# Jiraiya812/Fast-CU-Decision-HEVC

Measured on AMD Instinct MI355X. Metric: CTUs/sec (RDO decision only) at 4K all-intra, higher is better.
Workload: dtype int32+f64

## Files before the change

### fast-cu-decision-hevc_amd/csrc/fcu_engine.h

```cpp
#pragma once
#include <stdint.h>
#include <string.h>
#include <type_traits>
#include "../../include/fcu.h"

#ifdef FCU_EMU
#include <math.h>
#include <stdio.h>
#include <stdlib.h>
#define FCU_DEV static inline
#define FCU_MEMBER inline
#define FCU_NOINLINE
#define FCU_INLINE
#define FCU_TABLE static const
static int g_emu_phase = 0, g_emu_in_phase = 0, g_emu_lane = 0, g_emu_relax = 0;
#define FCU_EMU_RELAX(on) (g_emu_relax = (on))
static inline int fcu_emu_phase_begin() { g_emu_phase++; g_emu_in_phase = 1; g_emu_lane = 0; return 0; }
static inline int fcu_emu_phase_next(int lane) { if (lane + 1 >= 64) g_emu_in_phase = 0; g_emu_lane = lane + 1; return lane + 1; }
template <class T> static inline T fcu_emu_uni(T v, int site, int line)
{
  enum { SITES = 2048, K = 32, B = 16 };
  struct Seen { int phase, first, cur, idx, n; unsigned char vals[K][B]; };
  static Seen seen[SITES];
  if (g_emu_in_phase && !g_emu_relax && sizeof(T) <= B && site < SITES) {
// ... 37 lines not shown
  v += (uint32_t)__builtin_amdgcn_update_dpp(0, (int)v, 0x143, 0xc, 0xf, false);
  return (uint32_t)__builtin_amdgcn_readlane((int)v, 63);
}
__device__ inline unsigned long long fcu_wave_min64(unsigned long long v)
{
  for (int o = 32; o > 0; o >>= 1) {
    const unsigned lo = (unsigned)__shfl_xor((int)(unsigned)v, o), hi = (unsigned)__shfl_xor((int)(unsigned)(v >> 32), o);
    const unsigned long long w = ((unsigned long long)hi << 32) | lo;
    v = w < v ? w : v;
  }
  return v;
}
#define FCU_WAVE_ADD(p, v) do { const uint32_t s_ = fcu_wave_sum(v); if (threadIdx.x == 0) *(p) += s_; } while (0)
#define FCU_WAVE_MIN64(p, v) do { const unsigned long long s_ = fcu_wave_min64(v); if (threadIdx.x == 0 && s_ < *(p)) *(p) = s_; } while (0)
template <class T> __device__ inline T fcu_uni(T v)
{
  static_assert(sizeof(T) % 4 == 0, "dword-sized objects only");
  int w[sizeof(T) / 4];
  __builtin_memcpy(w, &v, sizeof(T));
  for (unsigned i = 0; i < sizeof(T) / 4; i++) w[i] = __builtin_amdgcn_readfirstlane(w[i]);
  __builtin_memcpy(&v, w, sizeof(T));
  return v;
}
#define FCU_UNI(x) fcu_uni(x)
#define FCU_EMU_RELAX(on) do { } while (0)
#if defined(__HIP_DEVICE_COMPILE__)
#define FCU_HBM __attribute__((address_space(1)))
#else
#define FCU_HBM
#endif
#define FCU_GENERIC_(p) ((const __attribute__((address_space(0))) void *)(p))
#define FCU_IN_LDS(p) __builtin_assume(__builtin_amdgcn_is_shared(FCU_GENERIC_(p)))
#define FCU_FLOOR(x) floor(x)
#define FCU_CHECK(c) do { } while (0)
#endif
#define FCU_DIST_ADD(acc, v, e, i, n2) do { \
    if ((n2) >= 64) { (acc) += (uint32_t)((e) * (e)); if (((((i) - lane) + 64) & ((n2) - 1)) == 0) { FCU_WAVE_ADD(&g_S.vc_dist[v], acc); (acc) = 0; } } \
    else FCU_ATOMIC_ADD(&g_S.vc_dist[v], (uint32_t)((e) * (e))); } while (0)
#define FCU_SERIAL FCU_FOR_LANES if (lane == 0)
#if defined(FCU_PROFILE) && !defined(FCU_EMU)
#define FCU_TIC(v) const long long v = clock64()
#ifdef FCU_PROFILE_RQT
#define FCU_QTIC(v) long long v = clock64()
#define FCU_QTOC(E_, v, idx) do { if (threadIdx.x == 0) (E_).C->prof[idx] += (unsigned long long)(clock64() - v); v = clock64(); } while (0)
#define FCU_TOC(E_, v, idx) do { if ((idx) == 10 && threadIdx.x == 0) (E_).C->prof[idx] += (unsigned long long)(clock64() - v); } while (0)
#define FCU_COUNT(E_, idx, n) do { } while (0)
#elif defined(FCU_PROFILE_INTER)
#define FCU_ITOC(E_, v, idx) do { if (threadIdx.x == 0) (E_).C->prof[idx] += (unsigned long long)(clock64() - v); } while (0)
#define FCU_TOC(E_, v, idx) do { if ((idx) == 10 && threadIdx.x == 0) (E_).C->prof[idx] += (unsigned long long)(clock64() - v); } while (0)
#define FCU_COUNT(E_, idx, n) do { } while (0)
#elif defined(FCU_PROFILE_RDOQ) || defined(FCU_PROFILE_DEPTH)
#define FCU_TOC(E_, v, idx) do { if ((idx) < 11 && threadIdx.x == 0) (E_).C->prof[idx] += (unsigned long long)(clock64() - v); } while (0)
#define FCU_COUNT(E_, idx, n) do { } while (0)
#else
#define FCU_TOC(E_, v, idx) do { if (threadIdx.x == 0) (E_).C->prof[idx] += (unsigned long long)(clock64() - v); } while (0)
#define FCU_COUNT(E_, idx, n) do { (E_).C->prof[idx] += (unsigned long long)(n); } while (0)
#endif
#else
#define FCU_TIC(v) do { } while (0)
#define FCU_TOC(E_, v, idx) do { } while (0)
#define FCU_COUNT(E_, idx, n) do { } while (0)
#endif
#ifndef FCU_QTOC
#define FCU_QTIC(v) do { } while (0)
#define FCU_QTOC(E_, v, idx) do { } while (0)
#endif
#ifndef FCU_ITOC
#define FCU_ITOC(E_, v, idx) do { } while (0)
#endif

#include "fcu_tables.h"

struct HotTables { uint32_t bin[256]; uint16_t scan[3][16]; uint8_t scan_cg8[3][4]; uint8_t ctx_ind_map4x4[16]; uint8_t group_idx[32];
                   uint64_t scan4_nib[3], map4_nib; uint32_t cnt_bits[4]; };
#ifdef FCU_EMU
static HotTables g_hot;
#else
__shared__ HotTables g_hot;
#endif

#if defined(FCU_PROFILE_RQT) && !defined(FCU_EMU)
#define FCU_RTIC(v) long long v = clock64()
#define FCU_RTOC(P_, v, idx) do { if (!SER && threadIdx.x == 0) { ((Chain *)((char *)&(P_) - __builtin_offsetof(Chain, p)))->prof[idx] += (unsigned long long)(clock64() - v); v = clock64(); } } while (0)
#elif defined(FCU_PROFILE_RDOQ) && !defined(FCU_EMU)
#define FCU_RTIC(v) long long v = clock64()
#define FCU_RTOC(P_, v, idx) do { if (SER) { ((Chain *)((char *)&(P_) - __builtin_offsetof(Chain, p)))->prof[idx] += (unsigned long long)(clock64() - v); v = clock64(); } } while (0)
#else
#define FCU_RTIC(v) do { } while (0)
#define FCU_RTOC(P_, v, idx) do { } while (0)
#endif
namespace fcu {

enum { CTU = 64, MAXDEPTH = 3, NPART = 256, LOG2_MAXTU = 5, LOG2_MINTU = 2, TU_MAXDEPTH_INTRA = 3 };
enum { SIZE_2Nx2N = 0, SIZE_2NxN = 1, SIZE_Nx2N = 2, SIZE_NxN = 3, SIZE_2NxnU = 4, SIZE_2NxnD = 5, SIZE_nLx2N = 6, SIZE_nRx2N = 7, SIZE_NONE = 8, MODE_INTER = 0, MODE_INTRA = 1, MODE_NONE = 2 };
enum { SLICE_I = 0, SLICE_P = 1 };
enum { PLANAR = 0, DC = 1, HOR = 10, VER = 26, DM_CHROMA = 36 };
enum { CTX_SPLIT = 0, CTX_PARTSIZE = 3, CTX_INTRA_LUMA = 4, CTX_CHROMA_PRED = 5, CTX_CBF_LUMA = 6, CTX_CBF_CHROMA = 11,
       CTX_SUBDIV = 16, CTX_SIGCG = 19, CTX_SIG = 23, CTX_LASTX = 67, CTX_LASTY = 97, CTX_ONE = 127, CTX_ABS = 151,
       CTX_TSKIP = 157, NCTX_INTRA = 160,
       CTX_SKIP = 160, CTX_MERGE_FLAG = 163, CTX_MERGE_IDX = 164, CTX_PRED_MODE = 165, CTX_PARTSIZE1 = 166, CTX_MVD = 169,
       CTX_REF = 171, CTX_MVP_IDX = 173, CTX_ROOT_CBF = 174, NCTX = 176 };
enum { CI_CURR_BEST = 0, CI_NEXT_BEST, CI_TEMP_BEST, CI_CHROMA_INTRA, CI_QT_TRAFO_TEST, CI_QT_TRAFO_ROOT, CI_NUM };
enum { MEMO_K = 6, MEMO_POOL = 6144 + 1536 + 384 + 96 };
enum { MAXVC = 20, MAXLC = 16, POOL = 5120 };
#define FCU_MAX_DOUBLE 1.7e+308

struct Cabac { uint8_t ctx[NCTX]; uint64_t frac; uint32_t bins; uint32_t pad_; };

struct Params {
  int width, height, qp, qp_c, slice_ctus, slice_type;
  int transform_skip, ts_fast, sign_hiding, strong_smoothing;
  double lambda, sqrt_lambda, chroma_weight, rdoq_lambda[3];
  double err_scale[2][4];
  long long rd_factor[2];
  int search_range, fast_enc, had_me, fdm, max_merge_cand, fast_search;
  int tmvp;
  int amp;
  int rdoq, rdoq_ts;
  uint32_t lambda_motion_sad;
  int cabac_b_table;
};
// ... 43 lines not shown
struct Yuv { uint8_t y[64 * 64], u[32 * 32], v[32 * 32]; };
enum { FCU_REF_MARGIN = 80 };
struct ChromaModeBuf { uint8_t u[32 * 32], v[32 * 32]; alignas(16) int16_t coef[2][1024]; uint8_t cbf[2][NPART], tskip[2][NPART]; };

struct RdoqRec { double cc, cs, c0; int32_t up, dn, sd, du; };

struct alignas(16) Scratch {
  CuObj cu[4][2];
  Yuv org[4], predt[4], reco[4][2];
  Yuv qt_rec[4];
  alignas(16) int16_t qt_coef[3][4][CTU * CTU];
  int16_t ts_coef[3][1024]; Yuv ts_rec; uint8_t shared_pred[3][1024];
  uint8_t tmp_tr_idx[NPART], tmp_cbf[NPART], tmp_tskip[NPART];
  ChromaModeBuf cm[5];
  Cabac slots[MAXDEPTH + 2][CI_NUM];
  uint8_t p_pred[POOL]; int16_t p_resi[POOL]; int32_t p_tmp[POOL]; int32_t p_tcoef[POOL]; uint8_t p_rec[POOL];
  int32_t p_lscan[POOL]; int16_t p_qscan[POOL];
  RdoqRec r_rec[POOL]; double r_cg[MAXVC * 64];
  uint8_t c64_rec[5][CTU * CTU]; alignas(16) int16_t c64_coef[5][CTU * CTU];
  Cabac c64_state[5][4]; uint32_t c64_distk[5][4];
  Yuv16 resi_cu, resi_best, qt_resi[4];
  Yuv tmp_pred;
  uint8_t me_pred[9][CTU * CTU];
  int16_t me_h[3][72 * 64];
  int par_ps[4];
  int memo_valid[4][MEMO_K], memo_next[4], memo_zero[4][MEMO_K];
  int16_t memo_mv[4][MEMO_K][NPART][2]; int8_t memo_ref[4][MEMO_K][NPART];
  uint8_t memo_tr_idx[4][MEMO_K][NPART], memo_cbf[4][MEMO_K][3][NPART], memo_tskip[4][MEMO_K][3][NPART];
  alignas(16) int16_t memo_coef[MEMO_K * MEMO_POOL], memo_resi[MEMO_K * MEMO_POOL];
};

struct Env { Chain *C; Scratch *G; int cur_ctu, slice_start; };
struct TU { int log2, tr_depth, part, nparts, x, y, off_y, cw, cwo, cx, cy, c_tr_depth, c_code_all, off_c, cu_depth, plast; };

struct Shared {
  Cabac cab[1 + (MAXDEPTH + 1) + MAXLC];
  uint8_t ref5[5][68]; int dc5[5]; uint32_t cm_dist[5];
  union {
    int16_t lane_abs[MAXLC][32];
    RdoqRec rq_rec[16];
    struct {
      int32_t colsum[128];
      union {
        struct { uint8_t ref[264], reff[264]; };
        uint8_t ref5b[5][68];
      };
    };
  };
  union {
    int16_t rq_lv[16];
    uint32_t sad[36];
  };
  int dc;
  int best_idx[4], reco_best_idx[4];
  union {
    struct { int rd_mode[12]; int n_rd; int preds[3]; int n_mpm; };
    int uni[8];
  };
  union {
    struct {
      uint8_t vc_slot[MAXVC];
      int vc_abs[MAXVC], vc_lsp[MAXVC], vc_last[MAXVC]; uint32_t vc_dist[MAXVC]; uint32_t vc_bits[MAXVC]; double vc_cost[MAXVC];
    };
    struct {
      uint32_t acc[16];
      unsigned long long me_best;
      int mrg_mv[5][2], mrg_ref[5], amvp[2][2];
      int iv_abs[6], iv_lsp[6], iv_top[6]; uint32_t iv_dist[6], iv_bits[6];
      int it_abs[3], it_ts[3]; uint32_t it_dist[3];
      double iq_cost[5]; uint32_t iq_bits[5], iq_dist[5], iq_zero;
      int16_t tz_x[16], tz_y[16]; uint8_t tz_pt[16], tz_d[16]; int tz_n;
      uint32_t tz_best; int tz_bx, tz_by, tz_dist, tz_round, tz_point;
      int mrg_buf[5], best_is_skip, me_out[4];
    };
  };
  int pu_best_vc, pu_best_mode, pu_nvc; uint32_t pu_best_dist; double pu_best_cost;
  int t_abs, t_lsp, t_last; uint32_t t_dist;
  int rw_abs, rw_lsp;
  double q_cost[4]; uint32_t q_dist[4];
  int c_best_mode; uint32_t c_best_dist; double c_best_cost; int c_modes[5];
  uint32_t c_dist;
  Env env;
  TU wk_st[4]; int wk_ci[4]; int wk_part[4], wk_child[4];
  double cand_cost[12];
  uint32_t c64_dist[5]; uint8_t c64_cbf[5][4]; int c64_valid;
  uint64_t q_frac[5], t_frac;
  double dec_j0, dec_j1; int dec_cnt, dec_flip;
};

enum { CAB_GOON = 0, CAB_CUR0 = 1, CAB_LANE0 = 1 + (MAXDEPTH + 1) };
enum { EST_CODERS = 7 };
static_assert(EST_CODERS * sizeof(Cabac) >= NCTX_INTRA * 2 * sizeof(uint32_t) && EST_CODERS <= MAXLC, "est table does not fit its lane coders");
#define FCU_EST ((uint32_t *)&g_S.cab[CAB_LANE0 + MAXLC - EST_CODERS])
#ifdef FCU_EMU
static Shared g_S;
#else
__shared__ Shared g_S;
#endif
FCU_DEV Env env_get() { return FCU_UNI(g_S.env); }
FCU_DEV Cabac *slot_ptr(const Env E, int d, int ci) { return ci == CI_CURR_BEST ? &g_S.cab[CAB_CUR0 + d] : &E.G->slots[d][ci]; }


FCU_DEV int part_x(int z) { return (k_z2r[z] & 15) << 2; }
FCU_DEV int part_y(int z) { return (k_z2r[z] >> 4) << 2; }
FCU_DEV int zidx_of(int lx, int ly) { return k_r2z[((ly & 63) >> 2) * 16 + ((lx & 63) >> 2)]; }
FCU_DEV int ilog2(int n) { int l = 0; while ((1 << l) < n) l++; return l; }
FCU_DEV int iabs(int v) { return v < 0 ? -v : v; }
FCU_DEV int clip8(int v) { return v < 0 ? 0 : (v > 255 ? 255 : v); }
FCU_DEV int clip3i(int lo, int hi, int v) { return v < lo ? lo : (v > hi ? hi : v); }
FCU_DEV uint8_t *yuv_plane(Yuv *b, int comp) { return comp == 0 ? b->y : (comp == 1 ? b->u : b->v); }
FCU_DEV double rd_cost(const Params &p, uint32_t bits, uint32_t dist)
{ return FCU_FLOOR((double)dist + ((double)bits * p.lambda) + 0.5); }

FCU_DEV void tu_root(TU &t, int depth)
{
  t.log2 = 6 - depth; t.tr_depth = 0; t.part = 0; t.nparts = NPART >> (2 * depth); t.x = t.y = 0; t.off_y = 0;
  t.cw = t.cwo = (CTU >> depth) >> 1; t.cx = t.cy = 0; t.c_tr_depth = 0; t.c_code_all = 1; t.off_c = 0;
  t.cu_depth = depth; t.plast = 0;
}
FCU_DEV void tu_child(TU &c, const TU &p, int i, int processLast)
{
  const int s = 1 << (p.log2 - 1);
  c.log2 = p.log2 - 1; c.tr_depth = p.tr_depth + 1; c.cu_depth = p.cu_depth; c.plast = processLast;
  c.nparts = p.nparts >> 2; if (c.nparts < 1) c.nparts = 1;
  c.part = p.part + i * c.nparts;
  c.x = p.x + (i & 1) * s; c.y = p.y + (i >> 1) * s; c.off_y = p.off_y + i * s * s;
  const int pw = p.cwo;
  if ((pw >> 1) >= 4) {
    const int cs = pw >> 1;
    c.cw = c.cwo = cs; c.c_code_all = 1; c.c_tr_depth = p.c_tr_depth + 1;
    c.cx = p.cx + (i & 1) * cs; c.cy = p.cy + (i >> 1) * cs; c.off_c = p.off_c + i * cs * cs;
  } else {
    c.cwo = pw; c.c_code_all = 0; c.c_tr_depth = p.c_tr_depth; c.cx = p.cx; c.cy = p.cy; c.off_c = p.off_c;
    c.cw = (processLast ? (i == 3) : (i == 0)) ? pw : 0;
  }
}
FCU_DEV uint32_t tu_key(const TU &t) { return (uint32_t)(t.cu_depth | (t.tr_depth << 2) | (t.part << 4) | (t.plast << 12)); }
FCU_DEV TU tu_of_key(uint32_t k)
{
  TU t; tu_root(t, (int)(k & 3));
  const int trd = (int)((k >> 2) & 3), part = (int)((k >> 4) & 255), pl = (int)((k >> 12) & 1);
  for (int l = 0; l < trd; l++) {
    TU c; int np = t.nparts >> 2; if (np < 1) np = 1;
    tu_child(c, t, ((part - t.part) / np) & 3, pl);
    t = c;
  }
// ... 916 lines not shown
  const int N = 1 << log2;
  const uint8_t *corner = ref + 2 * N;
  if (mode == PLANAR)
    return ((N - 1 - x) * corner[-1 - y] + (x + 1) * corner[1 + N] + (N - 1 - y) * corner[1 + x] + (y + 1) * corner[-1 - N] + N) >> (log2 + 1);
  if (mode == DC) {
    int v = dc;
    if (isLuma && N <= 16) {
      if (x == 0 && y == 0) v = (corner[1] + corner[-1] + 2 * dc + 2) >> 2;
      else if (y == 0) v = (corner[1 + x] + 3 * dc + 2) >> 2;
      else if (x == 0) v = (corner[-1 - y] + 3 * dc + 2) >> 2;
    }
    return v;
  }
  const int isVer = mode >= 18;
  const int angMode = isVer ? mode - VER : -(mode - HOR);
  const int absAng = iabs(angMode);
  const int angAbs = (int)((0x2069544d245080ull >> (6 * absAng)) & 63);
  const int invAngle = absAng == 0 ? 0 : (int)(((absAng <= 4 ? 0x13b0e38ccd000ull : 0x8004ec30c1e2ull) >> (13 * ((absAng - 1) & 3))) & 8191);
  const int angle = angMode < 0 ? -angAbs : angAbs;
  const int px = isVer ? x : y, py = isVer ? y : x, ms = isVer ? 1 : -1;
  if (angle == 0) {
    int v = corner[ms * (px + 1)];
    if (isLuma && N <= 16 && px == 0) v = clip8(v + ((corner[-ms * (py + 1)] - corner[0]) >> 1));
    return v;
  }
  const int deltaPos = (py + 1) * angle, di = deltaPos >> 5, df = deltaPos & 31;
  const int i0 = px + di + 1;
  int r0, r1;
  { int i = i0; r0 = (i >= 0) ? corner[ms * i] : corner[-ms * ((128 + (-i) * invAngle) >> 8)]; }
  if (!df) return r0;
  { int i = i0 + 1; r1 = (i >= 0) ? corner[ms * i] : corner[-ms * ((128 + (-i) * invAngle) >> 8)]; }
  return ((32 - df) * r0 + df * r1 + 16) >> 5;
}

FCU_DEV int unit_available(const Env E, int lx, int ly, int cx, int cy)
{
  const Params &P = E.C->p;
  if (lx < 0 || ly < 0 || lx >= P.width || ly >= P.height) return 0;
  const int ctuN = (ly >> 6) * E.C->w_ctu + (lx >> 6), ctuC = (cy >> 6) * E.C->w_ctu + (cx >> 6);
  if (ctuN < E.slice_start) return 0;
  if (ctuN < ctuC) return 1;
  if (ctuN > ctuC) return 0;
  return zidx_of(lx, ly) < zidx_of(cx, cy);
}

FCU_DEV FCU_NOINLINE void build_ref(int comp, int px, int py, int log2, int wantFilt)
{
  const Env E = env_get(); comp = FCU_UNI(comp); px = FCU_UNI(px); py = FCU_UNI(py); log2 = FCU_UNI(log2); wantFilt = FCU_UNI(wantFilt);
  const int N = 1 << log2, sh = comp ? 1 : 0, unit = 4 >> sh, total = 4 * N + 1;
  const int lx0 = px << sh, ly0 = py << sh;
  const uint8_t *rec = E.C->rec[comp]; const int stride = E.C->stride[comp];
  uint8_t *ref = g_S.ref, *avail = (uint8_t *)g_S.colsum;
  FCU_FOR_LANES {
    for (int i = lane; i < total; i += 64) {
      int a, v = 0;
      if (i < 2 * N) { const int y = 2 * N - 1 - i; a = unit_available(E, lx0 - 4, ((py + y) / unit * unit) << sh, lx0, ly0); if (a) v = rec[(py + y) * stride + px - 1]; }
      else if (i == 2 * N) { a = unit_available(E, lx0 - 4, ly0 - 4, lx0, ly0); if (a) v = rec[(py - 1) * stride + px - 1]; }
      else { const int x = i - 2 * N - 1; a = unit_available(E, ((px + x) / unit * unit) << sh, ly0 - 4, lx0, ly0); if (a) v = rec[(py - 1) * stride + px + x]; }
      avail[i] = (uint8_t)a; ref[i] = (uint8_t)v;
    }
  }
  FCU_FOR_LANES {
    for (int i = lane; i < total; i += 64) {
      if (!avail[i]) {
        int j = i - 1;
        while (j >= 0 && !avail[j]) j--;
        if (j < 0) { j = i + 1; while (j < total && !avail[j]) j++; }
        g_S.reff[i] = (j < total) ? ref[j] : 128;
      }
    }
  }
  FCU_FOR_LANES { for (int i = lane; i < total; i += 64) if (!avail[i]) ref[i] = g_S.reff[i]; }
  FCU_FOR_LANES {
    if (lane == 0) { int sum = 0; for (int i = 0; i < N; i++) sum += ref[2 * N + 1 + i] + ref[2 * N - 1 - i]; g_S.dc = (sum + N) >> (log2 + 1); }
    if (wantFilt) {
      int strong = 0;
      if (comp == 0 && E.C->p.strong_smoothing && N >= 32) {
        const int bl = ref[0], tl = ref[2 * N], tr = ref[4 * N];
        strong = (iabs(bl + tl - 2 * ref[N]) < 8) && (iabs(tl + tr - 2 * ref[3 * N]) < 8);
      }
      for (int i = lane; i < total; i += 64) {
        int v;
        if (i == 0 || i == 4 * N) v = ref[i];
        else if (strong) {
          const int bl = ref[0], tl = ref[2 * N], tr = ref[4 * N];
          if (i < 2 * N) v = ((2 * N - i) * bl + i * tl + N) >> (log2 + 1);
          else if (i == 2 * N) v = tl;
          else { const int k = i - 2 * N; v = ((2 * N - k) * tl + k * tr + N) >> (log2 + 1); }
        } else v = (ref[i - 1] + 2 * ref[i] + ref[i + 1] + 2) >> 2;
        g_S.reff[i] = (uint8_t)v;
      }
    }
  }
}

template <int N, class T>
FCU_DEV int32_t dot_row(const int8_t *m, const T *a)
{
  m = (const int8_t *)__builtin_assume_aligned(m, N >= 16 ? 16 : N);
  a = (const T *)__builtin_assume_aligned(a, sizeof(T) * N >= 16 ? 16 : 8);
  uint32_t mw[N / 4];
  __builtin_memcpy(mw, m, N);
  int32_t s = 0;
#pragma unroll
  for (int n = 0; n < N; n++) s += (int32_t)(int8_t)(mw[n >> 2] >> (8 * (n & 3))) * (int32_t)a[n];
  return s;
// ... 631 lines not shown
  st[0] = root; ci[0] = -1;
  while (sp >= 0) {
    const TU tu = st[sp];
    if (ci[sp] < 0) {
      if (cu->tr_idx[tu.part] == tu.tr_depth) {
        const int N = 1 << tu.log2, layer = LOG2_MAXTU - tu.log2;
        FCU_FOR_LANES {
          for (int i = lane; i < N * N; i += 64) {
            cu->coef[0][tu.off_y + i] = G->qt_coef[0][layer][tu.off_y + i];
            const int yy = tu.y + (i >> tu.log2), xx = tu.x + (i & (N - 1));
            reco->y[yy * 64 + xx] = G->qt_rec[layer].y[yy * 64 + xx];
          }
        }
        sp--; continue;
      }
      ci[sp] = 0;
    }
    if (ci[sp] >= 4) { sp--; continue; }
    { TU ch; tu_child(ch, st[sp], ci[sp], 0); ci[sp]++; sp++; st[sp] = ch; ci[sp] = -1; }
  }
}

template <int USZ>
FCU_DEV uint32_t satd_unit(const uint8_t *org, int log2, int mode, int dc, int bx, int by)
{
  const uint8_t *r = use_filtered_ref(mode, log2, 1) ? g_S.reff : g_S.ref;
  int acc[USZ * USZ];
#pragma unroll
  for (int i = 0; i < USZ * USZ; i++) acc[i] = 0;
  for (int y = 0; y < USZ; y++) {
    uint8_t o[USZ]; int row[USZ];
    __builtin_memcpy(o, org + (by + y) * 64 + bx, USZ);
#pragma unroll
    for (int x = 0; x < USZ; x++) row[x] = (int)o[x] - pred_pixel(r, log2, mode, 1, dc, bx + x, by + y);
#pragma unroll
    for (int len = 1; len < USZ; len <<= 1)
#pragma unroll
      for (int i = 0; i < USZ; i += 2 * len)
#pragma unroll
        for (int j = i; j < i + len; j++) { const int a = row[j], b = row[j + len]; row[j] = a + b; row[j + len] = a - b; }
#pragma unroll
    for (int k = 0; k < USZ; k++) {
      const int neg = -(__builtin_popcount((unsigned)(k & y)) & 1);
#pragma unroll
      for (int j = 0; j < USZ; j++) acc[k * USZ + j] += (row[j] ^ neg) - neg;
    }
  }
  int s = 0;
#pragma unroll
  for (int i = 0; i < USZ * USZ; i++) s += iabs(acc[i]);
  return (uint32_t)(USZ == 8 ? ((s + 2) >> 2) : ((s + 1) >> 1));
}

FCU_DEV FCU_NOINLINE void rmd(CuObj *cu, uint32_t tu_k)
{
  const Env E = env_get(); cu = FCU_UNI(cu); const TU tu = tu_of_key(FCU_UNI(tu_k));
  Scratch *G = E.G; const Params &P = E.C->p;
  const int d = cu->depth_cu, N = 1 << tu.log2, log2 = tu.log2;
  build_ref(0, cu->x + tu.x, cu->y + tu.y, log2, 1);
  const uint8_t *org = G->org[d].y + tu.y * 64 + tu.x;
  FCU_FOR_LANES { if (lane < 36) g_S.sad[lane] = 0; }
  FCU_FOR_LANES {
    const int dc = g_S.dc;
    if (N >= 8) {
      const int bpr = N >> 3, nblk = bpr * bpr;
      for (int u = lane; u < 35 * nblk; u += 64) { const int mode = u / nblk, blk = u - mode * nblk; FCU_ATOMIC_ADD(&g_S.sad[mode], satd_unit<8>(org, log2, mode, dc, (blk % bpr) * 8, (blk / bpr) * 8)); }
    } else {
      for (int u = lane; u < 35; u += 64) FCU_ATOMIC_ADD(&g_S.sad[u], satd_unit<4>(org, log2, u, dc, 0, 0));
    }
  }
  FCU_SERIAL {
    int preds[3];
    const int nm = intra_dir_predictor(E, cu, tu.part, preds);
    g_S.preds[0] = preds[0]; g_S.preds[1] = preds[1]; g_S.preds[2] = preds[2]; g_S.n_mpm = nm;
    const Cabac *cb = slot_ptr(E, d, CI_CURR_BEST);
    const uint64_t carry = cb->frac & 32767;
    int numFull = k_rd_mode_num[log2 - 2];
    double *candCost = g_S.cand_cost;
    for (int i = 0; i < numFull; i++) candCost[i] = FCU_MAX_DOUBLE;
    for (int mode = 0; mode < 35; mode++) {
      int predIdx = -1;
      for (int i = 0; i < 3; i++) if (mode == preds[i]) predIdx = i;
      const uint64_t fr = carry + (uint64_t)ctx_bits(CAB_CUR0 + d, CTX_INTRA_LUMA, predIdx != -1) + (uint64_t)32768 * (uint64_t)(predIdx != -1 ? (predIdx ? 2 : 1) : 5);
      const uint32_t modeBits = (uint32_t)(fr >> 15);
      const double cost = (double)g_S.sad[mode] + (double)modeBits * P.sqrt_lambda;
      int shift = 0;
      while (shift < numFull && cost < candCost[numFull - 1 - shift]) shift++;
      if (shift != 0) {
        for (int i = 1; i < shift; i++) { g_S.rd_mode[numFull - i] = g_S.rd_mode[numFull - 1 - i]; candCost[numFull - i] = candCost[numFull - 1 - i]; }
        g_S.rd_mode[numFull - shift] = mode; candCost[numFull - shift] = cost;
      }
    }
    for (int j = 0; j < nm; j++) {
      int inc = 0;
      for (int i = 0; i < numFull; i++) inc |= (preds[j] == g_S.rd_mode[i]);
      if (!inc) g_S.rd_mode[numFull++] = preds[j];
    }
    g_S.n_rd = numFull;
  }
}

FCU_DEV FCU_NOINLINE void pu_first_pass_batched(CuObj *cu, uint32_t tu_k)
{
  const Env E = env_get(); cu = FCU_UNI(cu); const TU tu = tu_of_key(FCU_UNI(tu_k));
  Scratch *G = E.G; const Params &P = E.C->p;
  const int d = cu->depth_cu, N = 1 << tu.log2, log2 = tu.log2, n2 = N * N, part = tu.part;
  const int partSize = cu->part_size[part];
  int checkTS = P.transform_skip && log2 == 2;
  if (P.ts_fast) checkTS = checkTS && (partSize == SIZE_NxN);
  const int nc = g_S.n_rd, tsv = checkTS ? 2 : 1, tss = tsv - 1, nvc = nc * tsv;
  FCU_CHECK(nvc <= MAXVC && nvc * n2 <= POOL && (MAXLC % 2) == 0);
  const int qbits = rdoq_qbits(log2, P.qp), qscale = k_quant_scales[P.qp % 6];
  const int useDst = log2 == 2;
  const uint8_t *org = G->org[d].y + tu.y * 64 + tu.x;
  build_ref(0, cu->x + tu.x, cu->y + tu.y, log2, 1);
  FCU_FOR_LANES {
    const int dc = g_S.dc;
    for (int i = lane; i < nc * n2; i += 64) {
      const int cnd = i / n2, p = i - cnd * n2, y = p >> log2, x = p & (N - 1), mode = g_S.rd_mode[cnd];
      const uint8_t *r = use_filtered_ref(mode, log2, 1) ? g_S.reff : g_S.ref;
      const int v = pred_pixel(r, log2, mode, 1, dc, x, y);
      G->p_pred[i] = (uint8_t)v; G->p_resi[i] = (int16_t)(org[y * 64 + x] - v);
    }
  }
  FCU_FOR_LANES { if (lane < nvc) g_S.vc_last[lane] = -1; by_log2(log2, [&](auto L) { constexpr int LG = decltype(L)::value; RowCache<(1 << LG), int16_t> rc; for (int i = lane; i < nc * n2; i += 64) { const int cnd = i / n2; G->p_tmp[i] = fwd1<LG>(rc, G->p_resi + cnd * n2, useDst, i - cnd * n2); } }); }
  FCU_FOR_LANES {
    est_build(CAB_CUR0 + d, lane);
    by_log2(log2, [&](auto L) { constexpr int LG = decltype(L)::value; RowCache<(1 << LG), int32_t> rc;
      for (int i = lane; i < nvc * n2; i += 64) {
        const int v = i / n2, p = i - v * n2, cnd = (v >> tss), ts = (v & tss);
        const uint16_t *iscan = k_iscan + k_scan_off[coef_scan_idx(g_S.rd_mode[cnd], log2, 0) * 4 + log2 - 2];
        const int32_t t = ts ? ((int32_t)G->p_resi[cnd * n2 + p] << (15 - 8 - log2)) : fwd2<LG>(rc, G->p_tmp + cnd * n2, useDst, p);
        const int sp = iscan[p]; const int32_t ld = level_double(t, qscale, qbits);
        G->p_lscan[sp * nvc + v] = ld;
        if (level_nonzero(ld, qbits)) FCU_ATOMIC_MAX(&g_S.vc_last[v], sp);
      }
    });
  }
  FCU_TIC(t2_);
  FCU_FOR_LANES {
    if (lane < nvc) {
      const int mode = g_S.rd_mode[(lane >> tss)];
      RdoqRec *rrec = G->r_rec + lane; double *rcg = G->r_cg + lane;
      const int cbfCtx = CTX_CBF_LUMA + (tu.tr_depth == 0 ? 1 : 0);
      const RdoqOut o = ((lane & tss) ? P.rdoq_ts : P.rdoq) ? rdoq<0, 1>(CAB_CUR0 + d, G->p_lscan + lane, G->p_qscan + lane, nvc, g_S.vc_last[lane], log2, 0, coef_scan_idx(mode, log2, 0), cbfCtx, P, rrec, rcg)
                                                            : quant_plain(G->p_lscan + lane, G->p_qscan + lane, nvc, g_S.vc_last[lane], log2, 0, P);
      g_S.vc_abs[lane] = o.abs_sum; g_S.vc_lsp[lane] = o.last;
      g_S.vc_dist[lane] = 0;
    }
    if (lane == 0) E.C->n_tu_trials += (unsigned long long)nvc;
  }
  FCU_TOC(E, t2_, 2);
  FCU_FOR_LANES {
    const DeqParams dq = deq_params(log2, P.qp);
    for (int i = lane; i < nvc * n2; i += 64) {
      const int v = i / n2, p = i - v * n2;
      const uint16_t *iscan = k_iscan + k_scan_off[coef_scan_idx(g_S.rd_mode[(v >> tss)], log2, 0) * 4 + log2 - 2];
      const int sp = iscan[p];
      const int q = (g_S.vc_abs[v] > 0 && (sp >> 4) <= (g_S.vc_last[v] >> 4)) ? G->p_qscan[sp * nvc + v] : 0;
      G->p_tmp[((v & tss)) ? i : v * n2 + tr_index(p, log2)] = dequant1(q, dq);
    }
  }
  FCU_FOR_LANES {
    by_log2(log2, [&](auto L) { constexpr int LG = decltype(L)::value; RowCache<(1 << LG), int32_t> rc;
      for (int i = lane; i < nvc * n2; i += 64) {
        const int v = i / n2, p = i - v * n2, ts = (v & tss);
        if (ts) { const int s = 15 - 8 - log2; G->p_tcoef[i] = (G->p_tmp[i] + (1 << (s - 1))) >> s; }
        else G->p_tcoef[i] = inv1<LG>(rc, G->p_tmp + v * n2, useDst, p);
      }
// ... 218 lines not shown
      for (int m = 0; m < nc; m++) {
        const int orgMode = g_S.rd_mode[m];
        FCU_FOR_LANES { for (int i = lane; i < tu.nparts; i += 64) cu->intra_dir[0][partOffset + i] = (uint8_t)orgMode; cab_copy(&g_S.cab[CAB_GOON], slot_ptr(E, d, CI_CURR_BEST), lane); if (lane == 0) { g_S.q_dist[0] = 0; g_S.q_cost[0] = 0; } }
        recur_luma_qt<0>(cu, tu_key(tu), 1);
        if (g_S.q_cost[0] < g_S.pu_best_cost) {
          FCU_SERIAL { g_S.pu_best_mode = orgMode; g_S.pu_best_dist = g_S.q_dist[0]; g_S.pu_best_cost = g_S.q_cost[0]; }
          set_intra_result_luma_qt(cu, tu_key(tu), recoT);
          FCU_FOR_LANES { for (int i = lane; i < tu.nparts; i += 64) { G->tmp_tr_idx[i] = cu->tr_idx[partOffset + i]; G->tmp_cbf[i] = cu->cbf[0][partOffset + i]; G->tmp_tskip[i] = cu->tskip[0][partOffset + i]; } }
        }
      }
    }
    if (log2 > min_tu_log2_in_cu(d, partSize)) {
      const int orgMode = g_S.pu_best_mode;
      FCU_FOR_LANES { for (int i = lane; i < tu.nparts; i += 64) cu->intra_dir[0][partOffset + i] = (uint8_t)orgMode; cab_copy(&g_S.cab[CAB_GOON], slot_ptr(E, d, CI_CURR_BEST), lane); if (lane == 0) { g_S.q_dist[0] = 0; g_S.q_cost[0] = 0; } }
      { FCU_TIC(t_); recur_luma_qt<0>(cu, tu_key(tu), 0, singleTU ? g_S.pu_best_vc : -1); FCU_TOC(E, t_, 4); }
      if (g_S.q_cost[0] < g_S.pu_best_cost) {
        FCU_SERIAL { g_S.pu_best_dist = g_S.q_dist[0]; g_S.pu_best_cost = g_S.q_cost[0]; }
        set_intra_result_luma_qt(cu, tu_key(tu), recoT);
        FCU_FOR_LANES { for (int i = lane; i < tu.nparts; i += 64) { G->tmp_tr_idx[i] = cu->tr_idx[partOffset + i]; G->tmp_cbf[i] = cu->cbf[0][partOffset + i]; G->tmp_tskip[i] = cu->tskip[0][partOffset + i]; } }
      }
    }
    overallDistY += g_S.pu_best_dist;
    const int bestMode = g_S.pu_best_mode;
    if (ptr) FCU_SERIAL { ptr->best_mode = (uint8_t)g_S.pu_best_mode; ptr->best_dist = g_S.pu_best_dist; ptr->best_cost = g_S.pu_best_cost; ptr->valid = 1; }
    FCU_FOR_LANES {
      for (int i = lane; i < tu.nparts; i += 64) {
        cu->tr_idx[partOffset + i] = G->tmp_tr_idx[i]; cu->cbf[0][partOffset + i] = G->tmp_cbf[i]; cu->tskip[0][partOffset + i] = G->tmp_tskip[i];
        cu->intra_dir[0][partOffset + i] = (uint8_t)bestMode;
      }
      if (pu != numPU - 1) {
        uint8_t *p = E.C->rec[0] + (cu->y + tu.y) * E.C->stride[0] + cu->x + tu.x; const int rs = E.C->stride[0];
        for (int i = lane; i < N * N; i += 64) p[(i >> log2) * rs + (i & (N - 1))] = recoT->y[(tu.y + (i >> log2)) * 64 + tu.x + (i & (N - 1))];
      }
    }
  }
  if (numPU > 1) {
    FCU_SERIAL {
      uint8_t cy = 0, cu1 = 0, cv = 0;
      for (int p = 0, idx = 0; p < 4; p++, idx += qNumParts) { cy |= (cu->cbf[0][idx] >> 1) & 1; cu1 |= (cu->cbf[1][idx] >> 1) & 1; cv |= (cu->cbf[2][idx] >> 1) & 1; }
      for (int o = 0; o < 4 * qNumParts; o++) { cu->cbf[0][o] |= cy; cu->cbf[1][o] |= cu1; cu->cbf[2][o] |= cv; }
    }
  }
  FCU_FOR_LANES { cab_copy(&g_S.cab[CAB_GOON], slot_ptr(E, d, CI_CURR_BEST), lane); if (lane == 0) cu->dist = overallDistY; }
}

FCU_DEV void chroma_leaf_refs5(const Env E, const CuObj *cu, int comp, int px, int py, int log2)
{
  Scratch *G = E.G;
  const int N = 1 << log2, total = 4 * N + 1, lx0 = px << 1, ly0 = py << 1;
  const uint8_t *rec = E.C->rec[comp]; const int stride = E.C->stride[comp];
  const int cx0 = cu->x >> 1, cy0 = cu->y >> 1, cs = (CTU >> cu->depth_cu) >> 1;
  uint8_t *avail = (uint8_t *)g_S.colsum;
  FCU_FOR_LANES {
    for (int i = lane; i < total; i += 64) {
      int a, x, y;
      if (i < 2 * N) { y = py + 2 * N - 1 - i; x = px - 1; a = unit_available(E, lx0 - 4, (y / 2 * 2) << 1, lx0, ly0); }
      else if (i == 2 * N) { y = py - 1; x = px - 1; a = unit_available(E, lx0 - 4, ly0 - 4, lx0, ly0); }
      else { x = px + i - 2 * N - 1; y = py - 1; a = unit_available(E, (x / 2 * 2) << 1, ly0 - 4, lx0, ly0); }
      avail[i] = (uint8_t)a;
      if (a) {
        const int inside = x >= cx0 && x < cx0 + cs && y >= cy0 && y < cy0 + cs;
        for (int m = 0; m < 5; m++) {
          const uint8_t *ov = comp == 1 ? G->cm[m].u : G->cm[m].v;
          g_S.ref5[m][i] = inside ? ov[(y - cy0) * 32 + (x - cx0)] : rec[y * stride + x];
        }
      }
    }
  }
  FCU_FOR_LANES {
    for (int i = lane; i < total; i += 64) {
      if (!avail[i]) {
        int j = i - 1;
        while (j >= 0 && !avail[j]) j--;
        if (j < 0) { j = i + 1; while (j < total && !avail[j]) j++; }
        for (int m = 0; m < 5; m++) g_S.ref5b[m][i] = (j < total) ? g_S.ref5[m][j] : 128;
      }
    }
  }
  FCU_FOR_LANES { for (int i = lane; i < total; i += 64) if (!avail[i]) for (int m = 0; m < 5; m++) g_S.ref5[m][i] = g_S.ref5b[m][i]; }
  FCU_FOR_LANES { if (lane < 5) { int sum = 0; for (int i = 0; i < N; i++) sum += g_S.ref5[lane][2 * N + 1 + i] + g_S.ref5[lane][2 * N - 1 - i]; g_S.dc5[lane] = (sum + N) >> (log2 + 1); } }
}

FCU_DEV FCU_NOINLINE uint32_t chroma_tree_bits(int c, const CuObj *cu, int m, int mode, int16_t *absbuf)
{
  const Env E = env_get(); cu = FCU_UNI(cu);
  FCU_IN_LDS(absbuf);
  const ChromaModeBuf *B = &E.G->cm[m];
  FCU_EMU_RELAX(1);
  cab_reset_bits(c);
  code_intra_dir_chroma(c, mode);
  TU *st = g_S.wk_st; int *ci = g_S.wk_ci;
  for (int pass = 0; pass < 3; pass++) {
    int sp = 0; tu_root(st[0], cu->depth_cu); ci[0] = -1;
    while (sp >= 0) {
      const TU tu = st[sp];
      if (ci[sp] < 0) {
        const int subdiv = cu->tr_idx[tu.part] > tu.tr_depth;
        if (pass == 0) {
          for (int k = 0; k < 2; k++)
            if (tu.c_code_all && (tu.tr_depth == 0 || ((B->cbf[k][tu.part] >> (tu.tr_depth - 1)) & 1))) {
              const int lowest = tu.tr_depth + ((subdiv && !(tu.cw >= 8)) ? 1 : 0);
              cab_bin(c, (B->cbf[k][tu_part_c(tu)] >> lowest) & 1, CTX_CBF_CHROMA + tu.tr_depth);
            }
        } else if (!subdiv) {
          const int k = pass - 1;
          if (tu.cw != 0 && ((B->cbf[k][tu.part] >> tu.tr_depth) & 1)) {
// ... 473 lines not shown
        sp--; continue;
      }
      stChild[sp] = 0;
    }
    if (stChild[sp] >= 4) { sp--; continue; }
    {
      const int qn = (NPART >> (2 * depth)) >> 2, p = part + stChild[sp] * qn;
      stChild[sp]++;
      if (ctu->x + part_x(p) < P.width && ctu->y + part_y(p) < P.height) { sp++; stPart[sp] = p; stChild[sp] = -1; }
    }
  }
}

FCU_DEV void load_hot_tables()
{
  FCU_FOR_LANES {
    for (int i = lane; i < 256; i += 64) g_hot.bin[i] = k_bin[i];
    for (int i = lane; i < 3 * 16; i += 64) { const int t = i / 16, j = i % 16; g_hot.scan[t][j] = k_scan[k_scan_off[t * 4 + 0] + j]; }
    if (lane < 12) g_hot.scan_cg8[lane / 4][lane % 4] = k_scan_cg[k_scan_cg_off[(lane / 4) * 4 + 1] + lane % 4];
    if (lane < 16) g_hot.ctx_ind_map4x4[lane] = k_ctx_ind_map4x4[lane];
    if (lane < 32) g_hot.group_idx[lane] = k_group_idx[lane];
    if (lane < 3) { uint64_t v = 0; for (int j = 0; j < 16; j++) v |= (uint64_t)k_scan[k_scan_off[lane * 4 + 0] + j] << (4 * j); g_hot.scan4_nib[lane] = v; }
    if (lane == 3) { uint64_t v = 0; for (int j = 0; j < 16; j++) v |= (uint64_t)k_ctx_ind_map4x4[j] << (4 * j); g_hot.map4_nib = v; }
    if (lane >= 4 && lane < 8) {
      const int pattern = lane - 4; uint32_t v = 0;
      for (int j = 0; j < 16; j++) {
        const int xs = j & 3, ys = j >> 2; int cnt;
        if (pattern == 0) { const int t = xs + ys; cnt = (t >= 3) ? 0 : ((t >= 1) ? 1 : 2); }
        else if (pattern == 1) cnt = (ys >= 2) ? 0 : ((ys >= 1) ? 1 : 2);
        else if (pattern == 2) cnt = (xs >= 2) ? 0 : ((xs >= 1) ? 1 : 2);
        else cnt = 2;
        v |= (uint32_t)cnt << (2 * j);
      }
      g_hot.cnt_bits[pattern] = v;
    }
  }
}

template <bool WPP = false>
FCU_DEV FCU_NOINLINE void compress_ctu(Chain *C, Scratch *G, int ctuRsAddr)
{
  C = FCU_UNI(C); G = FCU_UNI(G); ctuRsAddr = FCU_UNI(ctuRsAddr);
  Env E; E.C = C; E.G = G;
  FCU_TIC(t10_);
  const Params &P = C->p;
  const int sliceLen = P.slice_ctus > 0 ? P.slice_ctus : C->n_ctu;
  const int sliceStart = (ctuRsAddr / sliceLen) * sliceLen;
  int sliceEnd = sliceStart + sliceLen; if (sliceEnd > C->n_ctu) sliceEnd = C->n_ctu;
  E.cur_ctu = ctuRsAddr; E.slice_start = sliceStart;
  fcu_ctu_out *out = &C->out[ctuRsAddr];
  const int x = (ctuRsAddr % C->w_ctu) * CTU, y = (ctuRsAddr / C->w_ctu) * CTU;
  const int col = ctuRsAddr % C->w_ctu;
  const bool row_start = WPP && col == 0 && ctuRsAddr != sliceStart;
  FCU_SERIAL { g_S.env = E; if (ctuRsAddr == sliceStart || row_start) cab_init(slot_ptr(E, 0, CI_CURR_BEST), P.qp, P.slice_type, P.cabac_b_table); else cab_copy1(slot_ptr(E, 0, CI_CURR_BEST), &C->state); }
  if (row_start && C->w_ctu >= 2) {
    const uint8_t *src = C->wpp_sync_in;
    FCU_FOR_LANES { Cabac *d = slot_ptr(E, 0, CI_CURR_BEST); for (int i = lane; i < NCTX; i += 64) d->ctx[i] = src[i]; }
  }
  FCU_FOR_LANES {
    for (int i = lane; i < NPART; i += 64) {
      out->depth[i] = 0; out->width[i] = CTU; out->height[i] = CTU; out->skip[i] = 0; out->part_size[i] = SIZE_NONE; out->pred_mode[i] = MODE_NONE;
      out->tq_bypass[i] = 0; out->qp[i] = (int8_t)P.qp; out->chroma_qp_adj[i] = 0; out->tr_idx[i] = 0; out->ipcm[i] = 0;
      out->merge_flag[i] = 0; out->merge_idx[i] = 0; out->inter_dir[i] = 0; out->mvp_idx[i] = -1; out->ref_idx[i] = -1;
      out->mv[i][0] = out->mv[i][1] = 0; out->mvd[i][0] = out->mvd[i][1] = 0;
      for (int c = 0; c < 3; c++) { out->tskip[c][i] = 0; out->cbf[c][i] = 0; }
      out->intra_dir[0][i] = DC; out->intra_dir[1][i] = 0;
    }
    for (int i = lane; i < 4096; i += 64) out->coeff_y[i] = 0;
    for (int i = lane; i < 1024; i += 64) { out->coeff_cb[i] = 0; out->coeff_cr[i] = 0; }
    cab_copy(&g_S.cab[CAB_GOON], slot_ptr(E, 0, CI_CURR_BEST), lane);
    if (lane == 0) { for (int d = 0; d < 4; d++) { g_S.best_idx[d] = 0; g_S.reco_best_idx[d] = 0; } G->par_ps[0] = SIZE_NONE; out->total_cost = FCU_MAX_DOUBLE; out->total_dist = out->total_bits = out->total_bins = 0; }
  }
  cu_init(&G->cu[0][0], 0, x, y, 0);
  cu_init(&G->cu[0][1], 0, x, y, 0);
  compress_cu<0>();
  {
    const CuObj *view = cu_best(E, 0);
    FCU_FOR_LANES {
      cab_copy(&g_S.cab[CAB_GOON], slot_ptr(E, 0, CI_CURR_BEST), lane);
    }
    FCU_TIC(t9_);
    FCU_SERIAL {
      cab_reset_bits((CAB_GOON));
      encode_ctu((CAB_GOON), view, ctuRsAddr == sliceEnd - 1);
      cab_copy1(&C->state, &g_S.cab[CAB_GOON]);
    }
    FCU_TOC(E, t9_, 9);
    if (WPP && col == 1) {
      uint8_t *dst = C->wpp_sync_out;
      FCU_FOR_LANES { for (int i = lane; i < NCTX; i += 64) dst[i] = g_S.cab[CAB_GOON].ctx[i]; }
    }
  }
  FCU_TOC(E, t10_, 10);
}

enum { WPP_CTL_WORDS = 4, WPP_SYNC_BYTES = 192 };
#ifdef FCU_EMU
FCU_DEV bool wpp_wait(unsigned *ctl, int above, unsigned need) { FCU_CHECK(ctl[WPP_CTL_WORDS + above] >= need); return true; }
FCU_DEV void wpp_publish(unsigned *ctl, int chain, unsigned done) { ctl[WPP_CTL_WORDS + chain] = done; }
#else
#define FCU_WPP_GIVE_UP_TICKS (120ull * 100000000ull)
FCU_DEV bool wpp_wait(unsigned *ctl_, int above, unsigned need)
{
  FCU_HBM unsigned *ctl = (FCU_HBM unsigned *)ctl_;
  const unsigned long long t0 = __builtin_amdgcn_s_memrealtime();
  for (;;) {
    unsigned v = 0, ab = 0;
// ... 66 lines not shown
```

Measured before the change: 18570.

## Parallelize intra RMD SATD, mode ranking and reuse reference samples

Rough mode decision for 4x4 and 8x8 TUs now splits the work across lanes by (mode, line): each lane predicts one row, applies a 1D Hadamard, stages it in shared memory, and a second pass does the column transform. Candidate selection replaces the serial insertion sort with a parallel rank-by-comparison over 35 costs. A tag records the reference block, so the following first-pass PU evaluation skips rebuilding refs when the same TU was just prepared. The cost is extra shared-memory staging that aliases the lane CABAC coders, invalidation bookkeeping on the tag, and more complex prediction code whose tie-breaking must match the serial ordering.

```diff
diff --git a/fast-cu-decision-hevc_amd/csrc/fcu_engine.h b/fast-cu-decision-hevc_amd/csrc/fcu_engine.h
--- a/fast-cu-decision-hevc_amd/csrc/fcu_engine.h
+++ b/fast-cu-decision-hevc_amd/csrc/fcu_engine.h
@@ -113,6 +113,10 @@
 #elif defined(FCU_PROFILE_RDOQ) || defined(FCU_PROFILE_DEPTH)
 #define FCU_TOC(E_, v, idx) do { if ((idx) < 11 && threadIdx.x == 0) (E_).C->prof[idx] += (unsigned long long)(clock64() - v); } while (0)
 #define FCU_COUNT(E_, idx, n) do { } while (0)
+#elif defined(FCU_PROFILE_RMD)
+#define FCU_MTOC(E_, v, idx) do { if (threadIdx.x == 0) (E_).C->prof[idx] += (unsigned long long)(clock64() - v); } while (0)
+#define FCU_TOC(E_, v, idx) do { if ((idx) < 11 && threadIdx.x == 0) (E_).C->prof[idx] += (unsigned long long)(clock64() - v); } while (0)
+#define FCU_COUNT(E_, idx, n) do { } while (0)
 #else
 #define FCU_TOC(E_, v, idx) do { if (threadIdx.x == 0) (E_).C->prof[idx] += (unsigned long long)(clock64() - v); } while (0)
 #define FCU_COUNT(E_, idx, n) do { (E_).C->prof[idx] += (unsigned long long)(n); } while (0)
@@ -128,6 +132,9 @@
 #endif
 #ifndef FCU_ITOC
 #define FCU_ITOC(E_, v, idx) do { } while (0)
+#endif
+#ifndef FCU_MTOC
+#define FCU_MTOC(E_, v, idx) do { } while (0)
 #endif
 
 #include "fcu_tables.h"
@@ -277,6 +284,7 @@
     uint32_t sad[36];
   };
   int dc;
+  int ref_tag;
   int best_idx[4], reco_best_idx[4];
   union {
     struct { int rd_mode[12]; int n_rd; int preds[3]; int n_mpm; };
@@ -317,6 +325,11 @@
 enum { EST_CODERS = 7 };
 static_assert(EST_CODERS * sizeof(Cabac) >= NCTX_INTRA * 2 * sizeof(uint32_t) && EST_CODERS <= MAXLC, "est table does not fit its lane coders");
 #define FCU_EST ((uint32_t *)&g_S.cab[CAB_LANE0 + MAXLC - EST_CODERS])
+enum { RMD_STAGE_BYTES = 64 * 8 * 2, RMD_COST_BYTES = 35 * 8 };
+static_assert(RMD_STAGE_BYTES + RMD_COST_BYTES <= MAXLC * sizeof(Cabac) && (CAB_LANE0 * sizeof(Cabac)) % 8 == 0, "RMD staging does not fit the lane coders");
+#define FCU_RMD_STAGE ((int16_t *)&g_S.cab[CAB_LANE0])
+#define FCU_RMD_COST ((double *)((char *)&g_S.cab[CAB_LANE0] + RMD_STAGE_BYTES))
+FCU_DEV int ref_key(int px, int py, int log2) { return px | (py << 13) | (log2 << 26); }
 #ifdef FCU_EMU
 static Shared g_S;
 #else
@@ -1339,6 +1352,7 @@
   const uint8_t *rec = E.C->rec[comp]; const int stride = E.C->stride[comp];
   uint8_t *ref = g_S.ref, *avail = (uint8_t *)g_S.colsum;
   FCU_FOR_LANES {
+    if (lane == 0) g_S.ref_tag = -1;
     for (int i = lane; i < total; i += 64) {
       int a, v = 0;
       if (i < 2 * N) { const int y = 2 * N - 1 - i; a = unit_available(E, lx0 - 4, ((py + y) / unit * unit) << sh, lx0, ly0); if (a) v = rec[(py + y) * stride + px - 1]; }
@@ -2076,52 +2090,157 @@
   return (uint32_t)(USZ == 8 ? ((s + 2) >> 2) : ((s + 1) >> 1));
 }
 
+FCU_DEV int rmd_mode_of(int j) { return j < 2 ? j : j == 2 ? HOR : j == 3 ? VER : j < 12 ? j - 2 : j < 27 ? j - 1 : j; }
+
+template <int LOG2>
+FCU_DEV void pred_line(const uint8_t *ref, int mode, int dc, int line, int *out)
+{
+  constexpr int N = 1 << LOG2;
+  static_assert(N <= 8, "edge filters of DC / pure directions assumed on (N <= 16)");
+  const uint8_t *corner = ref + 2 * N;
+  if (mode < 2) {
+#pragma unroll
+    for (int k = 0; k < N; k++) out[k] = pred_pixel(ref, LOG2, mode, 1, dc, k, line);
+    return;
+  }
+  const int isVer = mode >= 18, ms = isVer ? 1 : -1;
+  const int angMode = isVer ? mode - VER : -(mode - HOR), absAng = iabs(angMode);
+  if (absAng == 0) {
+#pragma unroll
+    for (int k = 0; k < N; k++) out[k] = corner[ms * (k + 1)];
+    out[0] = clip8(out[0] + ((corner[-ms * (line + 1)] - corner[0]) >> 1));
+  } else {
+    const int angAbs = (int)((0x2069544d245080ull >> (6 * absAng)) & 63);
+    const int invAngle = (int)(((absAng <= 4 ? 0x13b0e38ccd000ull : 0x8004ec30c1e2ull) >> (13 * ((absAng - 1) & 3))) & 8191);
+    const int angle = angMode < 0 ? -angAbs : angAbs;
+    const int deltaPos = (line + 1) * angle, di = deltaPos >> 5, df = deltaPos & 31;
+    int r[N + 1];
+#pragma unroll
+    for (int k = 0; k <= N; k++) {
+      const int i = k + di + 1;
+      r[k] = (k == N && !df) ? 0 : (i >= 0) ? corner[ms * i] : corner[-ms * ((128 + (-i) * invAngle) >> 8)];
+    }
+#pragma unroll
+    for (int k = 0; k < N; k++) out[k] = df ? (((32 - df) * r[k] + df * r[k + 1] + 16) >> 5) : r[k];
+  }
+#ifdef FCU_EMU
+  for (int k = 0; k < N; k++) FCU_CHECK(out[k] == pred_pixel(ref, LOG2, mode, 1, dc, isVer ? k : line, isVer ? line : k));
+#endif
+}
+
+template <int N> FCU_DEV void hadamard_line(int *v)
+{
+#pragma unroll
+  for (int len = 1; len < N; len <<= 1)
+#pragma unroll
+    for (int i = 0; i < N; i += 2 * len)
+#pragma unroll
+      for (int j = i; j < i + len; j++) { const int a = v[j], b = v[j + len]; v[j] = a + b; v[j + len] = a - b; }
+}
+
+template <int LOG2>
+FCU_DEV void rmd_satd_small(const uint8_t *org)
+{
+  constexpr int N = 1 << LOG2, ITEMS = 35 * N;
+  int16_t *stage = FCU_RMD_STAGE;
+  for (int base = 0; base < ITEMS; base += 64) {
+    FCU_FOR_LANES {
+      const int it = base + lane;
+      if (it < ITEMS) {
+        const int mode = rmd_mode_of(it >> LOG2), line = it & (N - 1);
+        int v[N];
+        pred_line<LOG2>(use_filtered_ref(mode, LOG2, 1) ? g_S.reff : g_S.ref, mode, g_S.dc, line, v);
+        if (mode >= 2 && mode < 18) {
+#pragma unroll
+          for (int k = 0; k < N; k++) v[k] = (int)org[k * 64 + line] - v[k];
+        } else {
+          uint8_t o[N];
+          __builtin_memcpy(o, org + line * 64, N);
+#pragma unroll
+          for (int k = 0; k < N; k++) v[k] = (int)o[k] - v[k];
+        }
+        hadamard_line<N>(v);
+#pragma unroll
+        for (int k = 0; k < N; k++) stage[lane * N + k] = (int16_t)v[k];
+      }
+    }
+    FCU_FOR_LANES {
+      const int blk = lane >> LOG2, k = lane & (N - 1), it = base + blk * N;
+      if (it < ITEMS) {
+        int v[N];
+#pragma unroll
+        for (int l = 0; l < N; l++) v[l] = stage[(blk * N + l) * N + k];
+        hadamard_line<N>(v);
+        int sum = 0;
+#pragma unroll
+        for (int l = 0; l < N; l++) sum += iabs(v[l]);
+        FCU_ATOMIC_ADD(&g_S.sad[rmd_mode_of(it >> LOG2)], (uint32_t)sum);
+      }
+    }
+  }
+}
+
 FCU_DEV FCU_NOINLINE void rmd(CuObj *cu, uint32_t tu_k)
 {
   const Env E = env_get(); cu = FCU_UNI(cu); const TU tu = tu_of_key(FCU_UNI(tu_k));
   Scratch *G = E.G; const Params &P = E.C->p;
   const int d = cu->depth_cu, N = 1 << tu.log2, log2 = tu.log2;
-  build_ref(0, cu->x + tu.x, cu->y + tu.y, log2, 1);
+  { FCU_TIC(tm_); build_ref(0, cu->x + tu.x, cu->y + tu.y, log2, 1); FCU_MTOC(E, tm_, 11); }
   const uint8_t *org = G->org[d].y + tu.y * 64 + tu.x;
-  FCU_FOR_LANES { if (lane < 36) g_S.sad[lane] = 0; }
+  FCU_TIC(tm1_);
   FCU_FOR_LANES {
-    const int dc = g_S.dc;
-    if (N >= 8) {
+    if (lane < 36) g_S.sad[lane] = 0;
+    if (lane == 0) {
+      int preds[3];
+      g_S.n_mpm = intra_dir_predictor(E, cu, tu.part, preds);
+      g_S.preds[0] = preds[0]; g_S.preds[1] = preds[1]; g_S.preds[2] = preds[2];
+      g_S.ref_tag = ref_key(cu->x + tu.x, cu->y + tu.y, log2);
+    }
+  }
+  if (N >= 16) {
+    FCU_FOR_LANES {
+      const int dc = g_S.dc;
       const int bpr = N >> 3, nblk = bpr * bpr;
-      for (int u = lane; u < 35 * nblk; u += 64) { const int mode = u / nblk, blk = u - mode * nblk; FCU_ATOMIC_ADD(&g_S.sad[mode], satd_unit<8>(org, log2, mode, dc, (blk % bpr) * 8, (blk / bpr) * 8)); }
-    } else {
-      for (int u = lane; u < 35; u += 64) FCU_ATOMIC_ADD(&g_S.sad[u], satd_unit<4>(org, log2, u, dc, 0, 0));
-    }
-  }
-  FCU_SERIAL {
-    int preds[3];
-    const int nm = intra_dir_predictor(E, cu, tu.part, preds);
-    g_S.preds[0] = preds[0]; g_S.preds[1] = preds[1]; g_S.preds[2] = preds[2]; g_S.n_mpm = nm;
-    const Cabac *cb = slot_ptr(E, d, CI_CURR_BEST);
-    const uint64_t carry = cb->frac & 32767;
-    int numFull = k_rd_mode_num[log2 - 2];
-    double *candCost = g_S.cand_cost;
-    for (int i = 0; i < numFull; i++) candCost[i] = FCU_MAX_DOUBLE;
-    for (int mode = 0; mode < 35; mode++) {
+      for (int u = lane; u < 35 * nblk; u += 64) { const int j = u / nblk, blk = u - j * nblk, mode = rmd_mode_of(j); FCU_ATOMIC_ADD(&g_S.sad[mode], satd_unit<8>(org, log2, mode, dc, (blk % bpr) * 8, (blk / bpr) * 8)); }
+    }
+  } else if (N == 8) rmd_satd_small<3>(org);
+  else rmd_satd_small<2>(org);
+  FCU_MTOC(E, tm1_, 12);
+  FCU_TIC(tm2_);
+  const int numRmd = k_rd_mode_num[log2 - 2];
+  double *cost35 = FCU_RMD_COST;
+  FCU_FOR_LANES {
+    if (lane < 35) {
+      const int mode = lane;
       int predIdx = -1;
-      for (int i = 0; i < 3; i++) if (mode == preds[i]) predIdx = i;
+      for (int i = 0; i < 3; i++) if (mode == g_S.preds[i]) predIdx = i;
+      const uint64_t carry = slot_ptr(E, d, CI_CURR_BEST)->frac & 32767;
       const uint64_t fr = carry + (uint64_t)ctx_bits(CAB_CUR0 + d, CTX_INTRA_LUMA, predIdx != -1) + (uint64_t)32768 * (uint64_t)(predIdx != -1 ? (predIdx ? 2 : 1) : 5);
       const uint32_t modeBits = (uint32_t)(fr >> 15);
-      const double cost = (double)g_S.sad[mode] + (double)modeBits * P.sqrt_lambda;
-      int shift = 0;
-      while (shift < numFull && cost < candCost[numFull - 1 - shift]) shift++;
-      if (shift != 0) {
-        for (int i = 1; i < shift; i++) { g_S.rd_mode[numFull - i] = g_S.rd_mode[numFull - 1 - i]; candCost[numFull - i] = candCost[numFull - 1 - i]; }
-        g_S.rd_mode[numFull - shift] = mode; candCost[numFull - shift] = cost;
-      }
-    }
+      uint32_t sad = g_S.sad[mode];
+      if (N == 8) sad = (sad + 2) >> 2; else if (N == 4) sad = (sad + 1) >> 1;
+      cost35[mode] = (double)sad + (double)modeBits * P.sqrt_lambda;
+    }
+  }
+  FCU_FOR_LANES {
+    if (lane < 35) {
+      const double c = cost35[lane];
+      int rank = 0;
+      for (int m = 0; m < 35; m++) { const double o = cost35[m]; rank += (o < c || (o == c && m < lane)) ? 1 : 0; }
+      if (rank < numRmd) { g_S.rd_mode[rank] = lane; g_S.cand_cost[rank] = c; }
+    }
+  }
+  FCU_SERIAL {
+    int numFull = numRmd;
+    const int nm = g_S.n_mpm;
     for (int j = 0; j < nm; j++) {
       int inc = 0;
-      for (int i = 0; i < numFull; i++) inc |= (preds[j] == g_S.rd_mode[i]);
-      if (!inc) g_S.rd_mode[numFull++] = preds[j];
+      for (int i = 0; i < numFull; i++) inc |= (g_S.preds[j] == g_S.rd_mode[i]);
+      if (!inc) g_S.rd_mode[numFull++] = g_S.preds[j];
     }
     g_S.n_rd = numFull;
   }
+  FCU_MTOC(E, tm2_, 13);
 }
 
 FCU_DEV FCU_NOINLINE void pu_first_pass_batched(CuObj *cu, uint32_t tu_k)
@@ -2137,8 +2256,10 @@
   const int qbits = rdoq_qbits(log2, P.qp), qscale = k_quant_scales[P.qp % 6];
   const int useDst = log2 == 2;
   const uint8_t *org = G->org[d].y + tu.y * 64 + tu.x;
-  build_ref(0, cu->x + tu.x, cu->y + tu.y, log2, 1);
+  const int haveRefs = FCU_UNI(g_S.ref_tag) == ref_key(cu->x + tu.x, cu->y + tu.y, log2);
+  if (!haveRefs) { FCU_TIC(tm_); build_ref(0, cu->x + tu.x, cu->y + tu.y, log2, 1); FCU_MTOC(E, tm_, 14); }
   FCU_FOR_LANES {
+    if (lane == 0) g_S.ref_tag = -1;
     const int dc = g_S.dc;
     for (int i = lane; i < nc * n2; i += 64) {
       const int cnd = i / n2, p = i - cnd * n2, y = p >> log2, x = p & (N - 1), mode = g_S.rd_mode[cnd];
@@ -2463,6 +2584,7 @@
   const int cx0 = cu->x >> 1, cy0 = cu->y >> 1, cs = (CTU >> cu->depth_cu) >> 1;
   uint8_t *avail = (uint8_t *)g_S.colsum;
   FCU_FOR_LANES {
+    if (lane == 0) g_S.ref_tag = -1;
     for (int i = lane; i < total; i += 64) {
       int a, x, y;
       if (i < 2 * N) { y = py + 2 * N - 1 - i; x = px - 1; a = unit_available(E, lx0 - 4, (y / 2 * 2) << 1, lx0, ly0); }
@@ -3042,7 +3164,7 @@
   const int x = (ctuRsAddr % C->w_ctu) * CTU, y = (ctuRsAddr / C->w_ctu) * CTU;
   const int col = ctuRsAddr % C->w_ctu;
   const bool row_start = WPP && col == 0 && ctuRsAddr != sliceStart;
-  FCU_SERIAL { g_S.env = E; if (ctuRsAddr == sliceStart || row_start) cab_init(slot_ptr(E, 0, CI_CURR_BEST), P.qp, P.slice_type, P.cabac_b_table); else cab_copy1(slot_ptr(E, 0, CI_CURR_BEST), &C->state); }
+  FCU_SERIAL { g_S.env = E; g_S.ref_tag = -1; if (ctuRsAddr == sliceStart || row_start) cab_init(slot_ptr(E, 0, CI_CURR_BEST), P.qp, P.slice_type, P.cabac_b_table); else cab_copy1(slot_ptr(E, 0, CI_CURR_BEST), &C->state); }
   if (row_start && C->w_ctu >= 2) {
     const uint8_t *src = C->wpp_sync_in;
     FCU_FOR_LANES { Cabac *d = slot_ptr(E, 0, CI_CURR_BEST); for (int i = lane; i < NCTX; i += 64) d->ctx[i] = src[i]; }
```

New measurement: 19440, median of 6. 1.05x the previous value.
